# plus-rkwitt/flooder

Measured on AMD Instinct MI355X. Metric: M points×simplices/s (coverage sweep), higher is better.
Workload: dtype f32; 1 GPU; 1M-point 3D Gaussian, 1k landmarks, points_per_edge 30, max_dimension 3, fp32 coverage sweep (BASELINE.json configs[1]); points=1000000, landmarks=1000, top_simplices=6052, top_simplices_rank0=6052, swept_dimension=3, method=cell, parallelism=single GPU

## Files before the change

### flooder_amd/_native.py

```python

from __future__ import annotations

import ctypes
import os
from ctypes import c_char_p, c_float, c_int, c_int32, c_int64, c_uint32, c_void_p

_PKG_DIR = os.path.dirname(os.path.abspath(__file__))
LIB_PATH = os.environ.get("FLOODER_HIP_LIB") or os.path.join(_PKG_DIR, "libflooder_hip.so")



class _Block(ctypes.Structure):

    ABI = 1

    def __init__(self, **fields):
        super().__init__()
        self.size = ctypes.sizeof(self)
        self.abi = self.ABI
        known = {name for name, _ in self._fields_}
        for key, value in fields.items():
            if key not in known:
                raise TypeError(f"{type(self).__name__} has no field {key!r}")
            if value is not None and not isinstance(value, (int, float)):
# ... 8 lines not shown
        item = item.strip()
        if item:
            kind, name = item.split()
            out.append((name, kinds[kind]))
    return out


class FusedSweep(_Block):

    _fields_ = _fields("""u32 size; u32 abi; p pts_sorted; i64 n_pts; i32 dim; i32 k1; p nodes; p density_grid; p cloud_box;
        p verts; p weights; i32 R; i32 n_faces; i64 n_simplices; p memb; f32 alpha; i32 n_coarse; p coarse_rows; p parents;
        p face_bits; p face_slot; p d2_scratch; p flag_list; p flag_count; p flag_key; p flag_hist; p flag_sorted; p top;
        p top_list; p top_count; p simplex_weight; p plane_scratch; p wit_queue; p wit_item_list; p wit_stats;
        p cell_queue; p defer_list; p defer_c; p defer_ctl; p light_list; p heavy_list; p cell_stats; p finish_ctl;
        p hard_scratch; i32 hard_cap; i32 probed; p finish_stats; p wit_runs; i32 wit_run_len; i32 wit_n_runs;
        i32 planes_ready; i32 reserved""")


class SortedSweep(_Block):

    _fields_ = _fields("""u32 size; u32 abi; p pts_sorted; i64 n_pts; i32 dim; i32 k1; p nodes; p verts; p weights; i32 R;
        i32 n_faces; i64 n_simplices; p sample_order; p queue; p memb; p face_bits; p face_slot; p stats; p out_d2;
        i32 shard_rank; i32 shard_world""")


class FpsBatched(_Block):

    _fields_ = _fields("""u32 size; u32 abi; p pts; i64 n_pts; i32 dim; i32 ld; p pts_sorted; p order; i64 start; i32 n_lms;
        i32 reserved; p out_idx; p minsq; p bucket_box; p bucket_keys; p bucket_coord; p work_best; p work_rec; p work_ctr;
        p launches_out""")

# ... 102 lines not shown
                                             c_void_p]),
    "flooder_sweep_bvh_items_f32": (c_int, [c_void_p, c_int64, c_int, c_void_p, c_void_p, c_void_p, c_int, c_int,
                                            c_int64, c_void_p, c_void_p, c_void_p, c_void_p, c_int, c_void_p,
                                            c_void_p, c_void_p, c_void_p]),
    "flooder_sweep_cell_f32": (c_int, [c_void_p, c_int64, c_int, c_void_p, c_void_p, c_void_p, c_int, c_int,
                                       c_int64, c_float, c_void_p, c_void_p, c_void_p, c_void_p, c_void_p, c_void_p,
                                       c_void_p, c_void_p, c_void_p]),
    "flooder_density_grid_words": (c_int64, [c_int]),
    "flooder_density_grid_f32": (c_int, [c_void_p, c_int64, c_int, c_void_p, c_void_p, c_void_p]),
    "flooder_cloud_kind": (c_int, [c_void_p, c_int, c_void_p]),
    "flooder_wit_max_rows": (c_int, []),
    "flooder_wit_max_coarse": (c_int, []),
    "flooder_finish_single_tiles": (c_int, []),
    "flooder_finish_single_batches": (c_int, []),
    "flooder_face_values_f32": (c_int, [c_void_p, c_int64, c_void_p, c_void_p]),
    "flooder_simplex_weight_f32": (c_int, [c_void_p, c_int64, c_int, c_void_p, c_int, c_int64, c_void_p, c_void_p]),
    "flooder_simplex_planes_forget": (None, []),
    "flooder_simplex_prepare_f32": (c_int, [c_void_p, c_int64, c_int, c_void_p, c_int, c_int64, c_void_p, c_void_p, c_void_p,
                                            c_int64, c_void_p]),
    "flooder_selftest": (c_int, [c_void_p, c_void_p, c_void_p]),
    "flooder_fill_u32": (c_int, [c_void_p, c_int64, c_uint32, c_void_p]),
    "flooder_gather_rows_f64": (c_int, [c_void_p, c_int64, c_int, c_int, c_void_p, c_void_p, c_int64, c_void_p]),
    "flooder_sweep_bvh_f64": (c_int, [c_void_p, c_int64, c_int, c_void_p, c_void_p, c_void_p, c_int, c_int, c_int64,
                                      c_void_p, c_void_p, c_void_p]),
    "flooder_face_max_f64": (c_int, [c_void_p, c_int64, c_int, c_void_p, c_void_p, c_int, c_void_p, c_void_p, c_void_p]),
    "flooder_fps_bucket_count": (c_int64, [c_int64]),
    "flooder_fps_indexed_f32": (c_int, [c_void_p, c_int64, c_int, c_int, c_void_p, c_void_p, c_int, c_int64, c_void_p,
                                        c_void_p, c_void_p, c_void_p, c_void_p, c_void_p]),
    "flooder_fps_batched_max_points": (c_int64, []),
    "flooder_fps_batched_rec_words": (c_int64, [c_int64, c_int, c_int]),
# ... 108 lines not shown
```

### flooder_amd/core.py

```python

from __future__ import annotations

import ctypes
import itertools
import os
import weakref
import warnings
from numbers import Integral
from typing import Callable, Dict, List, NamedTuple, Optional, Tuple, Union

import numpy as np
import torch

from . import _native
from .simplex_tree import HAS_GUDHI, SimplexTree, delaunay_cells, delaunay_simplices

__all__ = ["flood_complex", "generate_landmarks", "generate_grid", "generate_uniform_weights",
           "SUPPORTED_DTYPES", "HAS_HIP_KERNELS", "PointIndex", "index_from_host"]

SUPPORTED_DTYPES = (torch.float32, torch.float64)
INF_BITS = 0x7F800000
CAND_ALIGN = 8
SWEEP_CHUNK = 2048
TILE_SAMPLES = 512
# ... 192 lines not shown
    n = simplex_vertices.shape[0]
    flat = torch.argmax(torch.cdist(simplex_vertices, simplex_vertices).flatten(1), dim=1)
    i0 = torch.div(flat, d + 1, rounding_mode="floor")
    i1 = flat - i0 * (d + 1)
    ar = torch.arange(n, device=simplex_vertices.device)
    centers = (simplex_vertices[ar, i0] + simplex_vertices[ar, i1]) / 2.0
    radii = torch.amax((simplex_vertices - centers.unsqueeze(1)).norm(dim=2), dim=1) \
        * (1.42 if d > 1 else 1.01) + 1e-3
    return centers, radii


_GRID_CACHE: Dict[tuple, tuple] = {}


def _grid_tables(points_per_edge: int, dim: int, device, dtype):
    key = (int(points_per_edge), int(dim), str(device), dtype, SAMPLE_UNITS)
    hit = _GRID_CACHE.get(key)
    if hit is None:
        weights, vertex_idxs, face_idxs = generate_grid(points_per_edge, dim, device, dtype)
        faces = _FaceTable(face_idxs, weights.shape[0], device)
        plan = SamplePlan(weights, faces) if torch.device(device).type == "cuda" else None
        v_np = [v.cpu().numpy() for v in vertex_idxs]
        if len(_GRID_CACHE) >= 16:
            _GRID_CACHE.clear()
        hit = _GRID_CACHE[key] = (weights, vertex_idxs, face_idxs, faces, plan, v_np)
    return hit


class _FaceTable:

    def __init__(self, face_idxs: Optional[List[torch.Tensor]], R: int, device):
# ... 496 lines not shown
        if n <= units[-1]:
            out.append(idx)
            continue
        P = X[idx]
        ax = int(np.argmax(P.max(axis=0) - P.min(axis=0)))
        idx = idx[np.argsort(P[:, ax], kind="stable")]
        unit = next((u for u in units if n > u), units[-1])
        n_left = (-(-n // unit) // 2) * unit
        if n_left <= 0 or n_left >= n:
            n_left = n // 2
        stack.append(idx[n_left:])
        stack.append(idx[:n_left])
    return np.concatenate(out)


WIT_MAX_COARSE = 256
WIT_MAX_ROWS = 8192
WIT_MIN_ROWS = 512
_WIT_PLAN_CACHE: Dict[tuple, Optional[tuple]] = {}


def witness_plan(weights: torch.Tensor, perm: np.ndarray) -> Optional[Tuple[np.ndarray, np.ndarray]]:
    w = weights.detach().cpu().numpy().astype(np.float64)
    R, k1 = w.shape
    if R < WIT_MIN_ROWS or R > WIT_MAX_ROWS or k1 < 2:
        return None
    key = (R, k1, hash(w.tobytes()), hash(np.asarray(perm).tobytes()))
    if key in _WIT_PLAN_CACHE:
        return _WIT_PLAN_CACHE[key]
    from scipy.spatial import cKDTree
# ... 68 lines not shown
    d = np.sqrt(((w - c64[:, None, :]) ** 2).sum(axis=2))
    rho = d.max(axis=1) * (1.0 + 1e-12)
    rho32 = rho.astype(np.float32)
    rho32 = np.where(rho32.astype(np.float64) < rho, np.nextafter(rho32, np.float32(np.inf)), rho32).astype(np.float32)
    sums = w32.astype(np.float64).sum(axis=1)
    if max(np.abs(sums - 1.0).max(), np.abs(c64.sum(axis=1) - 1.0).max()) > 0.5 * WIT_RUN_SUM_TOL:
        return None
    out = np.zeros((n, 8), dtype=np.uint32)
    out[:, :k1] = c32.view(np.uint32)
    out[:, 4] = np.bitwise_or.reduce(np.asarray(memb).view(np.uint32)[:n * run_len].reshape(n, run_len), axis=1)
    out[:, 5] = np.asarray(parents).view(np.uint32)[:n * run_len].reshape(n, run_len)[rows, d.argmin(axis=1)]
    out[:, 6] = rho32.view(np.uint32)
    return out


class SamplePlan:

    def __init__(self, weights: torch.Tensor, faces: _FaceTable):
        dev = weights.device
        self.R, self.k1 = weights.shape
        R = self.R
        perm = sample_order(weights)
        f_ptr = faces.ptr.cpu().numpy().astype(np.int64)
        f_rows = faces.rows.cpu().numpy().astype(np.int64)
        n_faces = faces.n_faces
        inv = np.empty(R, dtype=np.int64)
        inv[perm] = np.arange(R)
        self.inv = torch.as_tensor(inv, device=dev)
        self.w_perm = weights.to(torch.float32)[torch.as_tensor(perm, device=dev)].contiguous()
        self.rows_perm = self.inv[faces.rows.long()].to(torch.int32).contiguous()
        self.faces = faces
        self.memb_all = None
        if n_faces <= 32:
            memb_all = np.zeros(R, dtype=np.uint32)
            for f in range(n_faces):
                memb_all[inv[f_rows[f_ptr[f]:f_ptr[f + 1]]]] |= np.uint32(1 << f)
            self.memb_all = torch.as_tensor(memb_all.view(np.int32), device=dev)
        self._perm, self._weights, self._face_rows = perm, weights, (f_ptr, f_rows, inv)
        self._late_rows = self._wit = None
        self._late_built = self._wit_built = False
# ... 345 lines not shown
KNN_MERGE_WORKSPACE_BYTES = PROFILE_WORKSPACE_BYTES
SORTED_FUSED_FACES = False
BVH_SORTED_MIN_SAMPLES = 64 * 1024
EMPTY_CACHE_ABOVE_BYTES = 1 << 30
CELL_ALPHA = 1.35
FUSED_FACES = True
CELL_PROBE = True
SHARED_FACE_SLOTS = True
FINISH_HARD_CAP = 32768
CELL_DENSITY_GRID = True
CELL_SUPER = True
WIT_MIN_SIMPLICES = 1536
WIT_MAX_POINTS_PER_SIMPLEX = 400
CELL_WITNESS = True
WIT_RUNS = True


def _sweep_dimension_cell(index: PointIndex, verts: torch.Tensor, weights: torch.Tensor, faces: _FaceTable,
                          reduce_hook: Optional[Callable[[torch.Tensor], None]],
                          want_dist: bool = False, timer: Optional[_KernelTimer] = None,
                          stats: Optional[torch.Tensor] = None, plan: Optional[SamplePlan] = None,
                          face_slots: Optional[Tuple[torch.Tensor, int]] = None):
    lib = _native.load()
    dev = index.pts.device
    st = _native.current_stream_ptr(dev)
    S, k1, _ = verts.shape
    R = weights.shape[0]
    verts = verts.to(torch.float32).contiguous()
    plan = plan if plan is not None else SamplePlan(weights, faces)
    w_perm, rows_perm = plan.w_perm, plan.rows_perm
# ... 2 lines not shown
        return None if stats is None else stats[a:b]

    if S == 0:
        return (torch.empty((0, faces.n_faces), dtype=torch.float32, device=dev),
                torch.empty((0, R), dtype=torch.float32, device=dev) if want_dist else None)
    planes = torch.empty(24 * S, dtype=torch.float32, device=dev)
    if FUSED_FACES and not want_dist and reduce_hook is None and plan.memb_all is not None:
        F = faces.n_faces
        tiles = (R + 63) // 64
        slot_t, n_slots = face_slots if face_slots is not None else (None, S * F)
        CTL_FLAG_COUNT, CTL_DEFER, CTL_HIST = 1, 12, 48
        use_wit = (CELL_WITNESS and CELL_SUPER and CELL_PROBE and index.dim in (2, 3) and S >= WIT_MIN_SIMPLICES
                   and index.n <= WIT_MAX_POINTS_PER_SIMPLEX * S and plan.wit is not None)
        n_zeroed = ((1 if use_wit else 0) * QUEUE_WORDS + _native.CELL_QUEUE_WORDS + _native.FINISH_CTL_WORDS + 2 * S
                    + CTL_HIST + 8192 + n_slots)
        zeroed = (torch.empty if CELL_SUPER and SWEEP_PREPARE_FUSED else torch.zeros)(n_zeroed, dtype=torch.int32, device=dev)
        zeroed_all = zeroed
        if use_wit:
            qwit = zeroed[:QUEUE_WORDS]
            zeroed = zeroed[QUEUE_WORDS:]
        qbuf = zeroed[:_native.CELL_QUEUE_WORDS]
        fctl = zeroed[_native.CELL_QUEUE_WORDS:_native.CELL_QUEUE_WORDS + _native.FINISH_CTL_WORDS]
        zeroed = zeroed[_native.CELL_QUEUE_WORDS + _native.FINISH_CTL_WORDS:]
        top = zeroed[:2 * S].view(torch.int64)
        ctl = zeroed[2 * S:2 * S + CTL_HIST + 8192]
        face_bits = zeroed[2 * S + CTL_HIST + 8192:]
        hard = torch.empty(4 * FINISH_HARD_CAP, dtype=torch.int64, device=dev)
        top_list = torch.empty(S, dtype=torch.int32, device=dev)
        d2 = torch.empty((S, R), dtype=torch.int32, device=dev)
        flags = torch.empty((3, S * tiles), dtype=torch.int32, device=dev)
        chunks = (R + 255) // 256
        defer_list = torch.empty(5 * S * chunks, dtype=torch.int32, device=dev) if CELL_SUPER else None
        defer_c = torch.empty(5 * S * chunks, dtype=torch.float32, device=dev) if CELL_SUPER else None
        wgt = None
        split = torch.empty((2, S), dtype=torch.int32, device=dev) if CELL_SUPER else None
        if CELL_SUPER:
            wgt = torch.empty(S, dtype=torch.float32, device=dev)
            if SWEEP_PREPARE_FUSED:
                _native.check(lib.flooder_simplex_prepare_f32(_native.ptr(index.nodes), index.n, index.dim, _native.ptr(verts),
                                                              k1, S, _native.ptr(wgt), _native.ptr(planes),
                                                              _native.ptr(zeroed_all), n_zeroed, st),
# ... 4 lines not shown
        wst = stats[16:40] if use_wit and stats is not None and stats.numel() >= 40 else None
        blk = _native.FusedSweep(
            pts_sorted=index.pts, n_pts=index.n, dim=index.dim, k1=k1, nodes=index.nodes, density_grid=index.dens,
            cloud_box=index.box, verts=verts, weights=w_perm, R=R, n_faces=F, n_simplices=S, memb=plan.memb_all,
            alpha=float(CELL_ALPHA), face_bits=face_bits, face_slot=slot_t, d2_scratch=d2, flag_list=flags[0],
            flag_count=ctl[CTL_FLAG_COUNT:].data_ptr(), simplex_weight=wgt, plane_scratch=planes,
            cell_queue=qbuf.data_ptr(), defer_list=defer_list, defer_c=defer_c, cell_stats=sub(0, 9),
            finish_ctl=fctl.data_ptr(), hard_scratch=hard, hard_cap=FINISH_HARD_CAP, probed=1 if CELL_PROBE else 0,
            finish_stats=sub(9, 16))
        if CELL_PROBE:
            blk.flag_key, blk.flag_hist, blk.flag_sorted = flags[1].data_ptr(), ctl[CTL_HIST:].data_ptr(), flags[2].data_ptr()
            blk.top, blk.top_list = top.data_ptr(), top_list.data_ptr()
            blk.top_count = fctl[_native.FINISH_CTL_TOP_COUNT:].data_ptr()
        if CELL_SUPER:
            blk.defer_ctl, blk.light_list, blk.heavy_list = ctl[CTL_DEFER:].data_ptr(), split[0].data_ptr(), split[1].data_ptr()
        if use_wit:
            blk.n_coarse, blk.coarse_rows, blk.parents = plan.wit[2], plan.wit[0].data_ptr(), plan.wit[1].data_ptr()
            blk.wit_queue, blk.wit_item_list, blk.wit_stats = qwit.data_ptr(), split[0].data_ptr(), _native.ptr(wst) or None
            if WIT_RUNS and plan.wit_runs is not None:
                blk.wit_runs, blk.wit_run_len, blk.wit_n_runs = plan.wit_runs[0].data_ptr(), plan.wit_runs[1], plan.wit_runs[2]
        blk.planes_ready = 1 if CELL_SUPER and SWEEP_PREPARE_FUSED else 0
        with _span(timer, "sweep"):
            if use_wit:
                _native.check(lib.flooder_fused_witness(ctypes.byref(blk), st), "flooder_fused_witness")
                blk.planes_ready = 1
            _native.check(lib.flooder_fused_cell(ctypes.byref(blk), st), "flooder_fused_cell")
        with _span(timer, "fallback"):
            _native.check(lib.flooder_fused_finish(ctypes.byref(blk), st), "flooder_fused_finish")
        if stats is not None:
            c_d = ctl[CTL_DEFER:CTL_DEFER + _native.DEFER_CTL_WORDS].tolist()
            LAST_STATS.deferred_chunks = int(c_d[_native.DEFER_CTL_COUNT])
            LAST_STATS.light_heavy = (int(c_d[_native.DEFER_CTL_LIGHT]), int(c_d[_native.DEFER_CTL_HEAVY]))
            LAST_STATS.dense_tiles = int(c_d[_native.DEFER_CTL_TILE_COUNT])
            c_h = fctl[:_native.FINISH_CTL_QUEUES].tolist()
            LAST_STATS.hard_entries = (int(c_h[_native.FINISH_CTL_TOP_HARD_LEN]), int(c_h[_native.FINISH_CTL_REST_HARD_LEN]))
            LAST_STATS.finish_single_left = int(c_h[_native.FINISH_CTL_SINGLE_LEFT])
        out_face = torch.empty(n_slots if face_slots is not None else (S, F), dtype=torch.float32, device=dev)
        with _span(timer, "face_max"):
            _native.check(lib.flooder_face_values_f32(_native.ptr(face_bits), n_slots, _native.ptr(out_face), st),
                          "flooder_face_values_f32")
        return out_face, None

    ctl = torch.zeros(8 + 4 * QUEUE_WORDS, dtype=torch.int32, device=dev)
    qbuf = ctl[8:8 + 3 * QUEUE_WORDS]
    q_items = ctl[8 + 3 * QUEUE_WORDS:]
    d2 = torch.empty((S, R), dtype=torch.int32, device=dev)
    flags = torch.empty(S * ((R + 63) // 64), dtype=torch.int32, device=dev)
    with _span(timer, "sweep"):
        _native.check(lib.flooder_sweep_cell_f32(
            _native.ptr(index.pts), index.n, index.dim, _native.ptr(index.nodes), _native.ptr(verts),
            _native.ptr(w_perm), k1, R, S, float(CELL_ALPHA), qbuf.data_ptr(), _native.ptr(d2), _native.ptr(flags),
# ... 389 lines not shown
```

### flooder_amd/csrc/flood_cell.hip

```cpp

#include <type_traits>

#include "flood_common.hpp"
#include "flood_bvh.hpp"
#include "flood_planes.hpp"

using namespace flooder;

namespace {

constexpr int SPL_CHUNK = 4;
#ifndef FLOODER_CELL_CAPW
#define FLOODER_CELL_CAPW 480
#endif
#ifndef FLOODER_CELL_MAXLEAF
#define FLOODER_CELL_MAXLEAF 584
#endif
#ifndef FLOODER_CELL_WAVES
#define FLOODER_CELL_WAVES 4
#endif
#ifndef FLOODER_CELL_COMPACT
#define FLOODER_CELL_COMPACT 0
#endif
constexpr int CAPW = FLOODER_CELL_CAPW;
// ... 273 lines not shown
      const int gl = lfirst ? g : g - n_heavy_items;
      const int e = (TILES ? ARG(dl.tile_list) : ARG(dl.list))[gl];
      seeded = (e & 1) != 0;
      c_seed = (TILES ? ARG(dl.tile_c) : ARG(dl.c))[gl];
      s = (e >> 1) / chunks;
      q = (e >> 1) - s * chunks;
    } else {
      s = g / chunks;
      q = g - s * chunks;
    }
    s = wave_uniform(s);
    const int q_first = q;
    const float* vs = ARG(verts) + (int64_t)s * k1 * DIM;
    const int n_live = R;
    if (q * CHUNK >= n_live) continue;
    auto defer = [&](int qq, int seeded_flag, float c_next) {
      if (lane == 0) {
        const int pos = atomicAdd(ARG(dl.count), 1);
        ARG(dl.list)[pos] = (int)(((s * chunks + qq) << 1) | seeded_flag);
        ARG(dl.c)[pos] = c_next;
      }
    };
    PHASE(0);

    float p[SPL][DIM];
    float best[SPL];
    bool open[SPL];
    int row[SPL];
    float blo[DIM], bhi[DIM];
    auto make_samples = [&]() {
#pragma unroll
      for (int i = 0; i < SPL; ++i) {
        int slot = q * CHUNK + i * 64 + lane;
        open[i] = slot < n_live;
        if (slot >= n_live) slot = n_live - 1;
        const int r = slot;
        row[i] = r;
#pragma unroll
        for (int k = 0; k < DIM; ++k) p[i][k] = 0.f;
        if (k1 == 4) {
          const float4 w4 = *reinterpret_cast<const float4*>(weights + (int64_t)r * 4);
          const float wj[4] = {w4.x, w4.y, w4.z, w4.w};
#pragma unroll
          for (int j = 0; j < 4; ++j) {
#pragma unroll
            for (int k = 0; k < DIM; ++k) p[i][k] = __builtin_fmaf(wj[j], vs[j * DIM + k], p[i][k]);
          }
        } else {
          for (int j = 0; j < k1; ++j) {
            const float w = weights[(int64_t)r * k1 + j];
#pragma unroll
            for (int k = 0; k < DIM; ++k) p[i][k] = __builtin_fmaf(w, vs[j * DIM + k], p[i][k]);
// ... 24 lines not shown

    float slo[DIM + 1], shi[DIM + 1];
    {
      float mn[DIM], mx[DIM], dmn[DIM + 1], dmx[DIM + 1];
#pragma unroll
      for (int k = 0; k < DIM; ++k) { mn[k] = __builtin_inff(); mx[k] = -__builtin_inff(); }
#pragma unroll
      for (int f = 0; f <= DIM; ++f) { dmn[f] = __builtin_inff(); dmx[f] = -__builtin_inff(); }
      for (int sub = 0; sub < n_sub; ++sub) {
        q = q_first + sub;
        make_samples();
#pragma unroll
        for (int i = 0; i < SPL; ++i) {
#pragma unroll
          for (int k = 0; k < DIM; ++k) {
            mn[k] = __builtin_fminf(mn[k], p[i][k]);
            mx[k] = __builtin_fmaxf(mx[k], p[i][k]);
          }
#pragma unroll
          for (int f = 0; f <= DIM; ++f) {
            float dd = -po[f];
#pragma unroll
            for (int k = 0; k < DIM; ++k) dd = __builtin_fmaf(pn[f][k], p[i][k] - org[k], dd);
            dmn[f] = __builtin_fminf(dmn[f], dd);
            dmx[f] = __builtin_fmaxf(dmx[f], dd);
          }
        }
      }
#pragma unroll
      for (int k = 0; k < DIM; ++k) {
        blo[k] = wave_min_f32(mn[k]);
        bhi[k] = wave_max_f32(mx[k]);
      }
#pragma unroll
      for (int f = 0; f <= DIM; ++f) {
        slo[f] = wave_min_f32(dmn[f]);
        shi[f] = wave_max_f32(dmx[f]);
      }
    }
    float ext = 0.f, vol = 1.f;
// ... 158 lines not shown
    auto finalize = [&](bool seed_mode) {
    uint32_t* const out_d2 = ARG(out_d2);
    if (fused) {
      const FaceAcc acc = ARG(acc);
      uint32_t mb[SPL], um = 0u;
      bool fl_on[SPL];
      uint32_t fl_key[SPL];
#pragma unroll
      for (int i = 0; i < SPL; ++i) { fl_on[i] = false; fl_key[i] = 0u; }
      const int64_t my_slot = lane < acc.n_faces ? acc.slot_of(s, lane) : 0;
      const uint32_t my_fb = lane < acc.n_faces
                                 ? __hip_atomic_load(acc.face_bits + my_slot, __ATOMIC_RELAXED, __HIP_MEMORY_SCOPE_AGENT)
                                 : 0xffffffffu;
#pragma unroll
      for (int i = 0; i < SPL; ++i) {
        const bool settled = (q * CHUNK + i * 64 + lane < n_live) && !open[i];
        mb[i] = settled ? acc.memb[row[i]] : 0u;
        um |= mb[i];
      }
      um = wave_or_u32(um);
      while (um) {
        const int f = __builtin_ctz(um);
        um &= um - 1u;
        uint32_t v = 0u;
#pragma unroll
        for (int i = 0; i < SPL; ++i) {
          const uint32_t b = ((mb[i] >> f) & 1u) ? __float_as_uint(best[i]) : 0u;
          v = b > v ? b : v;
        }
        v = wave_max_u32(v);
        if (lane == f && v > my_fb) atomicMax(&acc.face_bits[my_slot], v);
// ... 869 lines not shown
int launch_simplex_planes(int dim, const float* verts, int k1, int64_t n_simplices, float* tab, hipStream_t st) {
  if (dim == 2)
    hipLaunchKernelGGL((simplex_planes_kernel<2>), dim3((unsigned)((n_simplices + 255) / 256)), dim3(256), 0, st, verts, k1,
                       n_simplices, tab);
  else if (dim == 3)
    hipLaunchKernelGGL((simplex_planes_kernel<3>), dim3((unsigned)((n_simplices + 255) / 256)), dim3(256), 0, st, verts, k1,
                       n_simplices, tab);
  else
    return fail(FLOODER_E_ARG, "simplex planes: only dim 2 and 3");
  return check_launch("simplex_planes");
}
}

namespace {

__global__ __launch_bounds__(1024) void split_simplices_kernel(const float* __restrict__ weight, int n, float limit,
                                                               float sparse_limit, int32_t* __restrict__ light,
                                                               int32_t* __restrict__ heavy, int32_t* __restrict__ counts) {
  __shared__ int s_cl[16], s_ch[16];
  __shared__ int s_sparse, s_act;
  const int lane = threadIdx.x & 63, wv = threadIdx.x >> 6;
  if (threadIdx.x == 0) { s_sparse = 0; s_act = 0; }
  __syncthreads();
  int mine = 0, act = 0;
  for (int i = threadIdx.x; i < n; i += 1024) {
    const float w = weight[i];
    mine += (w >= 0.f && w <= sparse_limit) ? 1 : 0;
    act += w >= 0.f ? 1 : 0;
  }
#pragma unroll
  for (int o = 32; o > 0; o >>= 1) {
    mine += __shfl_xor(mine, o);
    act += __shfl_xor(act, o);
// ... 21 lines not shown
    if (is_heavy) heavy[n_heavy + bh + __builtin_amdgcn_mbcnt_hi((uint32_t)(mh >> 32), __builtin_amdgcn_mbcnt_lo((uint32_t)mh, 0))] = i;
    n_light += tl;
    n_heavy += th;
    __syncthreads();
  }
  if (threadIdx.x == 0) { counts[0] = n_light; counts[1] = n_heavy; counts[2] = 1; }
}

constexpr int SPLIT_THREADS_LONG = 512;
constexpr int SPLIT_THREADS = 256;
constexpr int SPLIT_CLASSES = 9;
template <int NT>
__global__ __launch_bounds__(NT) void class_order_kernel(const float* __restrict__ weight, int n, float limit,
                                                               float sparse_limit, int runs_allowed, int reorder,
                                                               int32_t* __restrict__ light, int32_t* __restrict__ heavy,
                                                               int32_t* __restrict__ counts) {
  __shared__ int s_cnt[NT / 64][SPLIT_CLASSES + 1];
  constexpr int ID_LDS = 7680;
  __shared__ int s_id[ID_LDS];
  if (reorder) {
    n = counts[1];
    if (n > ID_LDS || n < 2 || counts[0] == 0) return;
    for (int i = threadIdx.x; i < n; i += NT) s_id[i] = heavy[i];
    __syncthreads();
  }
  constexpr int W_LDS = 7680;
  __shared__ float s_w[W_LDS];
  const bool staged = n <= W_LDS;
  if (staged) {
    for (int base = 0; base < n; base += NT * 8) {
      float v[8];
// ... 163 lines not shown
}

int flooder::fused_cell(const flooder_fused_sweep_t& a, void* stream) {
  if (a.n_simplices == 0 || a.R == 0) return FLOODER_OK;
  if (!a.memb || !a.face_bits || a.n_faces < 1 || a.n_faces > 32 || (a.top && (!a.top_list || !a.top_count)) ||
      (a.defer_list && (!a.defer_c || !a.defer_ctl)) ||
      (a.simplex_weight && (!a.defer_list || !a.light_list || !a.heavy_list)) || (a.flag_key && (!a.flag_hist || !a.top)) ||
      a.n_simplices > 0x7fffffffLL)
    return fail(FLOODER_E_ARG, "flooder_sweep_cell_faces_f32: bad argument");
  const float* const weight = a.simplex_weight;
  int32_t* const light = weight ? a.light_list : nullptr;
  int32_t* const heavy = weight ? a.heavy_list : nullptr;
  int32_t* const split = weight ? a.defer_ctl + FLOODER_DEFER_CTL_LIGHT : nullptr;
  const int n = (int)a.n_simplices;
  const hipStream_t st = (hipStream_t)stream;
  if (weight) {
    const bool long_queue = a.n_simplices * (int64_t)((a.R + 255) / 256) >= (int64_t)g_cell_super_min_chunks;
    if (long_queue && (g_cell_split_launches == 2 || a.n_simplices > 7680)) {
      hipLaunchKernelGGL(split_simplices_kernel, dim3(1), dim3(1024), 0, st, weight, n, (float)g_cell_super_weight,
                         (float)g_cell_super_sparse, light, heavy, split);
      if (g_cell_weight_classes)
        hipLaunchKernelGGL(class_order_kernel<SPLIT_THREADS>, dim3(1), dim3(SPLIT_THREADS), 0, st, weight, n,
                           (float)g_cell_super_weight, (float)g_cell_super_sparse, 2, 1, light, heavy, split);
    } else if (long_queue) {
      hipLaunchKernelGGL(class_order_kernel<SPLIT_THREADS_LONG>, dim3(1), dim3(SPLIT_THREADS_LONG), 0, st, weight, n,
                         (float)g_cell_super_weight, (float)g_cell_super_sparse, (g_cell_weight_classes ? 2 : 0) | 1 | 4, 0,
                         light, heavy, split);
    } else {
      hipLaunchKernelGGL(class_order_kernel<SPLIT_THREADS>, dim3(1), dim3(SPLIT_THREADS), 0, st, weight, n,
                         (float)g_cell_super_weight, (float)g_cell_super_sparse, g_cell_weight_classes ? 2 : 0, 0, light,
                         heavy, split);
    }
  }
  DeferList dl{a.defer_list, a.defer_c, a.defer_list ? a.defer_ctl + FLOODER_DEFER_CTL_COUNT : nullptr, light, heavy,
               split, g_cell_super_n0};
  if (a.defer_list) {
    const int64_t n_chunk_slots = a.n_simplices * (int64_t)((a.R + 255) / 256);
    dl.tile_list = a.defer_list + n_chunk_slots;
    dl.tile_c = a.defer_c + n_chunk_slots;
    dl.tile_count = a.defer_ctl + FLOODER_DEFER_CTL_TILE_COUNT;
  }
  return sweep_cell_entry(a,
                          FaceAcc{a.memb, a.face_bits, a.n_faces, reinterpret_cast<unsigned long long*>(a.top), a.top_list,
                                  a.top_count, a.face_slot, a.flag_key, a.flag_hist},
                          dl, "flooder_sweep_cell_faces_f32: bad argument", stream);
}

extern "C" {

int flooder_sweep_cell_f32(const float* pts_sorted, int64_t n_pts, int dim, const float* nodes,
                           const float* verts, const float* weights, int k1, int R, int64_t n_simplices,
                           float alpha, int32_t* queue, uint32_t* out_d2, int32_t* flag_list, int32_t* flag_count,
                           float* plane_scratch, const int32_t* density_grid, const float* cloud_box, uint64_t* stats,
                           void* stream) {
  flooder_fused_sweep_t a{};
  a.pts_sorted = pts_sorted; a.n_pts = n_pts; a.dim = dim; a.nodes = nodes; a.verts = verts; a.weights = weights;
  a.k1 = k1; a.R = R; a.n_simplices = n_simplices; a.alpha = alpha; a.cell_queue = queue; a.d2_scratch = out_d2;
  a.flag_list = flag_list; a.flag_count = flag_count; a.plane_scratch = plane_scratch; a.density_grid = density_grid;
  a.cloud_box = cloud_box; a.cell_stats = stats;
  return sweep_cell_entry(a, FaceAcc{nullptr, nullptr, 0, nullptr, nullptr, nullptr, nullptr},
// ... 56 lines not shown
```

### flooder_amd/csrc/flood_common.hpp

```cpp
#pragma once
#include <hip/hip_runtime.h>
#include <stdint.h>
#include <stdio.h>
#include <string.h>

#include "../../include/flooder_hip.h"

namespace flooder {

constexpr uint32_t INF_BITS = 0x7f800000u;

#define FLOODER_OPTION(name, def, lo, hi, desc) extern int g_##name;
#define FLOODER_OPTION_LIST(name, def, desc, ...) extern int g_##name;
#include "flood_options.def"
#undef FLOODER_OPTION
#undef FLOODER_OPTION_LIST
int launch_simplex_planes(int dim, const float* verts, int k1, int64_t n_simplices, float* tab, hipStream_t st);
char* err_buf();
int fail(int code, const char* msg);
int check_launch(const char* what);

__host__ __device__ constexpr int padded_dim(int dim) { return dim <= 2 ? 2 : (dim <= 4 ? 4 : 8); }

template <int DP>
// ... 162 lines not shown
  x |= dpp_move_u32<0x143, 0xC>(x);
  return (uint32_t)__builtin_amdgcn_readlane((int)x, 63);
}

constexpr uint32_t SETTLED_BIT = 0x80000000u;
struct FaceAcc {
  const uint32_t* memb;
  uint32_t* face_bits;
  int n_faces;
  unsigned long long* top;
  int32_t* top_list;
  int32_t* top_count;
  const int32_t* slot;
  uint32_t* flag_key = nullptr;
  int32_t* flag_hist = nullptr;
  __device__ __forceinline__ int64_t slot_of(int64_t s, int f) const {
    return slot ? (int64_t)slot[s * (int64_t)n_faces + f] : s * (int64_t)n_faces + f;
  }
};

template <template <int> class F, typename... Args>
int dispatch_dim(int dim, Args&&... args) {
  switch (dim) {
    case 1: return F<1>::run(args...);
    case 2: return F<2>::run(args...);
    case 3: return F<3>::run(args...);
    case 4: return F<4>::run(args...);
    case 5: return F<5>::run(args...);
    case 6: return F<6>::run(args...);
    case 7: return F<7>::run(args...);
    case 8: return F<8>::run(args...);
    default: return fail(FLOODER_E_ARG, "dim must be in 1..8");
  }
}
// ... 90 lines not shown
```

### flooder_amd/csrc/flood_finish.hip

```cpp

#include "flood_common.hpp"
#include "flood_bvh.hpp"
#include "flood_planes.hpp"

using namespace flooder;

namespace {

constexpr int SHORT_LIST = 1024;
#ifndef FLOODER_TOP_NODES
#define FLOODER_TOP_NODES 1024
#endif
#ifndef FLOODER_FINISH_PRIO_AFTER
#define FLOODER_FINISH_PRIO_AFTER 32
#endif
#ifndef FLOODER_FINISH_PRIO
#define FLOODER_FINISH_PRIO 3
#endif
#ifndef FLOODER_FINISH_WAVES
#define FLOODER_FINISH_WAVES 4
#endif
constexpr int TOP_NODES = FLOODER_TOP_NODES;

struct HardLists {
// ... 702 lines not shown
    const int c = s_cnt[b];
    if (c > 0) s_base[b] += atomicAdd(&cursor[b], c);
    s_cnt[b] = 0;
  }
  __syncthreads();
  for (int i = i0 + threadIdx.x; i < i1; i += 256) {
    const int b = (int)(flag_key[i] >> 19);
    flag_sorted[s_base[b] + atomicAdd(&s_cnt[b], 1)] = flag_list[i];
  }
}

__global__ void face_values_kernel(const uint32_t* __restrict__ bits, int64_t n, float* __restrict__ out) {
  const int64_t stride = (int64_t)gridDim.x * blockDim.x;
  for (int64_t i = (int64_t)blockIdx.x * blockDim.x + threadIdx.x; i < n; i += stride)
    out[i] = __builtin_sqrtf(__uint_as_float(bits[i]));
}

template <int DIM>
struct FinishOp {
  static int run(const flooder_fused_sweep_t& a, const Levels& lv, FaceAcc acc, hipStream_t st) {
    if constexpr (DIM != 2 && DIM != 3) {
      return fail(FLOODER_E_ARG, "flooder_finish_faces_f32: only dim 2 and 3");
    } else {
    int32_t* const ctl = a.finish_ctl;
    const int hard_cap = a.hard_cap;
    unsigned long long* top = reinterpret_cast<unsigned long long*>(a.top);
    unsigned long long* hard = reinterpret_cast<unsigned long long*>(a.hard_scratch);
    unsigned long long* stats = reinterpret_cast<unsigned long long*>(a.finish_stats);
    const int grid = g_bvh_grid;
    const bool wide = g_finish_wide_points > 0 && lv.count[0] * (int64_t)FLOODER_BVH_LEAF >= (int64_t)g_finish_wide_points;
// ... 92 lines not shown
  a.flag_sorted = flag_sorted; a.finish_ctl = ctl; a.top = top; a.top_list = top_list; a.probed = probed;
  a.d2_scratch = d2_scratch; a.memb = memb; a.n_faces = n_faces; a.face_bits = face_bits; a.face_slot = face_slot;
  a.hard_scratch = hard_scratch; a.hard_cap = hard_cap; a.finish_stats = stats;
  return fused_finish(a, stream);
}

int flooder_face_values_f32(const uint32_t* face_bits, int64_t n, float* out_face, void* stream) {
  if (n == 0) return FLOODER_OK;
  if (!face_bits || !out_face || n < 0) return fail(FLOODER_E_ARG, "flooder_face_values_f32: bad argument");
  int64_t blocks = (n + 255) / 256;
  if (blocks > 2048) blocks = 2048;
  hipLaunchKernelGGL(face_values_kernel, dim3((int)blocks), dim3(256), 0, (hipStream_t)stream, face_bits, n, out_face);
  return check_launch("face_values");
}

}

namespace {

constexpr int WFRONT = 256;

template <int DIM>
__global__ __launch_bounds__(256) void simplex_weight_kernel(const float* __restrict__ nodes, Levels lv,
                                                             const float* __restrict__ verts, int k1,
                                                             int64_t n_simplices, float* __restrict__ weight,
                                                             int weight_blocks, float* __restrict__ plane_tab,
                                                             int32_t* __restrict__ zero_buf, int64_t zero_words) {
  constexpr int DP = padded_dim(DIM);
  __shared__ int s_front[4][2][WFRONT];
  const int lane = threadIdx.x & 63, wv = threadIdx.x >> 6;
// ... 117 lines not shown
```

### include/flooder_hip.h

```cpp
#ifndef FLOODER_HIP_H
#define FLOODER_HIP_H

#include <stdint.h>

#ifdef __cplusplus
extern "C" {
#endif

#define FLOODER_ABI_VERSION 1

#define FLOODER_OK 0
#define FLOODER_E_ARG (-1)
#define FLOODER_E_LAUNCH (-2)
#define FLOODER_E_DEVICE (-3)

#define FLOODER_MAX_DIM 8
#define FLOODER_MAX_VERTS 9
#define FLOODER_CAND_ALIGN 8
#define FLOODER_SWEEP_CHUNK 2048
#define FLOODER_TILE_SAMPLES 512
#define FLOODER_BVH_LEAF 16
#define FLOODER_BVH_FANOUT 64
#define FLOODER_BVH_MAX_LEVELS 6
#define FLOODER_QUEUE_SHARDS 16
// ... 156 lines not shown
#define FLOODER_FINISH_CTL_WORDS (FLOODER_FINISH_CTL_QUEUES + 3 * FLOODER_QUEUE_WORDS)
#define FLOODER_DEFER_CTL_COUNT 0
#define FLOODER_DEFER_CTL_QUEUE 1
#define FLOODER_DEFER_CTL_LIGHT 2
#define FLOODER_DEFER_CTL_HEAVY 3
#define FLOODER_DEFER_CTL_SPLIT_DONE 4
#define FLOODER_DEFER_CTL_TILE_COUNT 6
#define FLOODER_DEFER_CTL_WORDS 8
#define FLOODER_CELL_QUEUE_RUNS 0
#define FLOODER_CELL_QUEUE_CHUNKS FLOODER_QUEUE_WORDS
#define FLOODER_CELL_QUEUE_TILES (2 * FLOODER_QUEUE_WORDS)
#define FLOODER_CELL_QUEUE_WORDS (3 * FLOODER_QUEUE_WORDS)
#define FLOODER_WIT_QUEUE_ITEM_COUNT (FLOODER_QUEUE_WORDS - 1)

int flooder_face_values_f32(const uint32_t* face_bits, int64_t n, float* out_face, void* stream);

int flooder_simplex_weight_f32(const float* nodes, int64_t n_pts, int dim, const float* verts, int k1,
                               int64_t n_simplices, float* weight, void* stream);

int flooder_simplex_prepare_f32(const float* nodes, int64_t n_pts, int dim, const float* verts, int k1,
                                int64_t n_simplices, float* weight, float* plane_scratch, int32_t* zero_buf,
                                int64_t zero_words, void* stream);
void flooder_simplex_planes_forget(void);

int flooder_selftest(const float* in64, float* out128, void* stream);

int flooder_fill_u32(uint32_t* buf, int64_t n, uint32_t value, void* stream);

int flooder_fps_f32(const float* pts, int64_t n_pts, int dim, int ld, int n_lms, int64_t start,
                    int64_t* out_idx, float* work_min, uint64_t* work_best, void* stream);
// ... 60 lines not shown
  float* defer_c;
  int32_t* defer_ctl;
  int32_t* light_list;
  int32_t* heavy_list;
  uint64_t* cell_stats;
  int32_t* finish_ctl;
  uint64_t* hard_scratch;
  int32_t hard_cap;
  int32_t probed;
  uint64_t* finish_stats;
  const uint32_t* wit_runs;
  int32_t wit_run_len;
  int32_t wit_n_runs;
  int32_t planes_ready;
  int32_t reserved;
} flooder_fused_sweep_t;

int flooder_fused_witness(const flooder_fused_sweep_t* p, void* stream);
int flooder_fused_cell(const flooder_fused_sweep_t* p, void* stream);
int flooder_fused_finish(const flooder_fused_sweep_t* p, void* stream);

typedef struct flooder_sorted_sweep_s {
  uint32_t size, abi;
  const float* pts_sorted;
  int64_t n_pts;
  int32_t dim;
  int32_t k1;
  const float* nodes;
  const float* verts;
  const float* weights;
// ... 154 lines not shown
```

Baseline: 6.217 million M points×simplices/s.

## Assign shared faces to one owner simplex and skip non-owned face samples

Grid rows are grouped by the smallest face that contains them. Each shared face gets a single owner simplex, chosen by atomicMax on a weight-based key inside the existing split/class-order launches. The cell sweep masks out rows on faces a simplex does not own and skips whole chunks or tiles that hold no owned faces. A new face-closure kernel then propagates maxima from sub-faces, so each face value still covers all of its boundary samples. This is meant to cut redundant sampling of faces shared between neighbouring simplices, at the cost of an owner pass, extra per-chunk mask loads and one more kernel.

```diff
diff --git a/flooder_amd/_native.py b/flooder_amd/_native.py
--- a/flooder_amd/_native.py
+++ b/flooder_amd/_native.py
@@ -46,7 +46,7 @@
         p top_list; p top_count; p simplex_weight; p plane_scratch; p wit_queue; p wit_item_list; p wit_stats;
         p cell_queue; p defer_list; p defer_c; p defer_ctl; p light_list; p heavy_list; p cell_stats; p finish_ctl;
         p hard_scratch; i32 hard_cap; i32 probed; p finish_stats; p wit_runs; i32 wit_run_len; i32 wit_n_runs;
-        i32 planes_ready; i32 reserved""")
+        i32 planes_ready; i32 reserved; p face_owner; p min_face; p chunk_faces; p tile_faces""")
 
 
 class SortedSweep(_Block):
@@ -179,6 +179,7 @@
     "flooder_finish_single_tiles": (c_int, []),
     "flooder_finish_single_batches": (c_int, []),
     "flooder_face_values_f32": (c_int, [c_void_p, c_int64, c_void_p, c_void_p]),
+    "flooder_face_closure_f32": (c_int, [c_void_p, c_void_p, c_void_p, c_int64, c_int, c_void_p, c_void_p]),
     "flooder_simplex_weight_f32": (c_int, [c_void_p, c_int64, c_int, c_void_p, c_int, c_int64, c_void_p, c_void_p]),
     "flooder_simplex_planes_forget": (None, []),
     "flooder_simplex_prepare_f32": (c_int, [c_void_p, c_int64, c_int, c_void_p, c_int, c_int64, c_void_p, c_void_p, c_void_p,
diff --git a/flooder_amd/core.py b/flooder_amd/core.py
--- a/flooder_amd/core.py
+++ b/flooder_amd/core.py
@@ -230,7 +230,7 @@
 
 
 def _grid_tables(points_per_edge: int, dim: int, device, dtype):
-    key = (int(points_per_edge), int(dim), str(device), dtype, SAMPLE_UNITS)
+    key = (int(points_per_edge), int(dim), str(device), dtype, SAMPLE_UNITS, bool(FACE_OWNER), bool(FACE_OWNER_GROUPED))
     hit = _GRID_CACHE.get(key)
     if hit is None:
         weights, vertex_idxs, face_idxs = generate_grid(points_per_edge, dim, device, dtype)
@@ -757,6 +757,56 @@
     return np.concatenate(out)
 
 
+def sample_order_grouped(weights: np.ndarray, group: np.ndarray) -> np.ndarray:
+    w = np.asarray(weights, dtype=np.float64)
+    R, k1 = w.shape
+    corners = np.eye(k1) - 1.0 / k1
+    X = w @ (corners @ np.linalg.qr(corners.T)[0][:, :k1 - 1])
+    out: List[np.ndarray] = []
+    pos = 0
+    for g in np.unique(group):
+        stack = [(np.nonzero(group == g)[0].astype(np.int64), pos)]
+        while stack:
+            idx, a = stack.pop()
+            n = idx.shape[0]
+            if n <= SAMPLE_UNITS[-1]:
+                out.append(idx)
+                continue
+            P = X[idx]
+            ax = int(np.argmax(P.max(axis=0) - P.min(axis=0)))
+            idx = idx[np.argsort(P[:, ax], kind="stable")]
+            n_left = n // 2
+            for u in SAMPLE_UNITS:
+                k0, k1_ = a // u + 1, -(-(a + n) // u) - 1
+                if k1_ >= k0:
+                    n_left = (k0 + (k1_ - k0 + 2) // 2 - 1) * u - a
+                    break
+            stack.append((idx[n_left:], a + n_left))
+            stack.append((idx[:n_left], a))
+        pos += int((group == g).sum())
+    return np.concatenate(out) if out else np.arange(R, dtype=np.int64)
+
+
+def row_groups(min_face: np.ndarray, sub_faces: np.ndarray, n_per_codim: List[int]) -> np.ndarray:
+    n1 = n_per_codim[1] if len(n_per_codim) > 1 else 0
+    group = min_face.astype(np.int64).copy()
+    small = group > n1
+    if small.any():
+        inside = (sub_faces[1:n1 + 1, None].astype(np.int64) >> min_face[None, small].astype(np.int64)) & 1
+        group[small] = 1 + inside.argmax(axis=0)
+    return group
+
+
+def _grouped_order_cached(w: np.ndarray, group: np.ndarray) -> np.ndarray:
+    key = (w.shape, hash(w.tobytes()), hash(group.tobytes()), SAMPLE_UNITS, "grouped")
+    hit = _SAMPLE_ORDER_CACHE.get(key)
+    if hit is None:
+        if len(_SAMPLE_ORDER_CACHE) >= 32:
+            _SAMPLE_ORDER_CACHE.clear()
+        hit = _SAMPLE_ORDER_CACHE[key] = sample_order_grouped(w, group)
+    return hit.copy()
+
+
 WIT_MAX_COARSE = 256
 WIT_MAX_ROWS = 8192
 WIT_MIN_ROWS = 512
@@ -855,6 +905,34 @@
     return out
 
 
+def face_lattice(weights: np.ndarray, f_ptr: np.ndarray, f_rows: np.ndarray) -> Optional[Tuple[np.ndarray, np.ndarray]]:
+    w = np.asarray(weights)
+    R, k1 = w.shape
+    F = len(f_ptr) - 1
+    if F > 32 or k1 > 31:
+        return None
+    supp = ((w != 0) * (1 << np.arange(k1))).sum(axis=1).astype(np.int64)
+    vset = np.array([np.bitwise_or.reduce(supp[f_rows[f_ptr[f]:f_ptr[f + 1]]]) if f_ptr[f + 1] > f_ptr[f] else 0
+                     for f in range(F)], dtype=np.int64)
+    if len(set(vset.tolist())) != F or (vset == 0).any():
+        return None
+    holds = (supp[:, None] & ~vset[None, :]) == 0
+    if not holds.any(axis=1).all():
+        return None
+    size = np.array([bin(int(v)).count("1") for v in vset])
+    min_face = np.where(holds, size[None, :], k1 + 1).argmin(axis=1).astype(np.uint8)
+    sub = (vset[None, :] & ~vset[:, None]) == 0
+    sub_faces = (sub * (1 << np.arange(F, dtype=np.int64))[None, :]).sum(axis=1).astype(np.uint32)
+    return min_face, sub_faces
+
+
+def _or_runs(bits: np.ndarray, run: int) -> np.ndarray:
+    n = (bits.shape[0] + run - 1) // run
+    pad = np.zeros(n * run, dtype=np.uint32)
+    pad[:bits.shape[0]] = bits
+    return np.bitwise_or.reduce(pad.reshape(n, run), axis=1)
+
+
 class SamplePlan:
 
     def __init__(self, weights: torch.Tensor, faces: _FaceTable):
@@ -865,6 +943,23 @@
         f_ptr = faces.ptr.cpu().numpy().astype(np.int64)
         f_rows = faces.rows.cpu().numpy().astype(np.int64)
         n_faces = faces.n_faces
+        self.min_face = self.chunk_faces = self.tile_faces = self.sub_faces = self.row_group = None
+        self.owner_order = False
+        if FACE_OWNER and n_faces <= 32 and self.k1 <= 8:
+            w_np = weights.detach().cpu().numpy()
+            lat = face_lattice(w_np, f_ptr, f_rows)
+            if lat is not None:
+                min_face, sub_faces = lat
+                if FACE_OWNER_GROUPED and len(f_ptr) > 2:
+                    group = row_groups(min_face, sub_faces, faces.n_per_codim)
+                    perm = _grouped_order_cached(w_np, group)
+                    self.row_group = group[perm]
+                bits = np.left_shift(np.uint32(1), min_face[perm].astype(np.uint32))
+                self.min_face = torch.as_tensor(np.ascontiguousarray(min_face[perm]), device=dev)
+                self.chunk_faces = torch.as_tensor(_or_runs(bits, 256).view(np.int32), device=dev)
+                self.tile_faces = torch.as_tensor(_or_runs(bits, 64).view(np.int32), device=dev)
+                self.sub_faces = torch.as_tensor(sub_faces.view(np.int32), device=dev)
+                self.owner_order = True
         inv = np.empty(R, dtype=np.int64)
         inv[perm] = np.arange(R)
         self.inv = torch.as_tensor(inv, device=dev)
@@ -1240,6 +1335,8 @@
 WIT_MAX_POINTS_PER_SIMPLEX = 400
 CELL_WITNESS = True
 WIT_RUNS = True
+FACE_OWNER = True
+FACE_OWNER_GROUPED = False
 
 
 def _sweep_dimension_cell(index: PointIndex, verts: torch.Tensor, weights: torch.Tensor, faces: _FaceTable,
@@ -1272,6 +1369,11 @@
                    and index.n <= WIT_MAX_POINTS_PER_SIMPLEX * S and plan.wit is not None)
         n_zeroed = ((1 if use_wit else 0) * QUEUE_WORDS + _native.CELL_QUEUE_WORDS + _native.FINISH_CTL_WORDS + 2 * S
                     + CTL_HIST + 8192 + n_slots)
+        use_owner = (FACE_OWNER and face_slots is not None and plan.owner_order and CELL_SUPER and SWEEP_PREPARE_FUSED
+                     and plan.sub_faces.numel() == F)
+        n_plain = n_zeroed
+        if use_owner:
+            n_zeroed += (n_zeroed & 1) + 3 * n_slots
         zeroed = (torch.empty if CELL_SUPER and SWEEP_PREPARE_FUSED else torch.zeros)(n_zeroed, dtype=torch.int32, device=dev)
         zeroed_all = zeroed
         if use_wit:
@@ -1282,7 +1384,8 @@
         zeroed = zeroed[_native.CELL_QUEUE_WORDS + _native.FINISH_CTL_WORDS:]
         top = zeroed[:2 * S].view(torch.int64)
         ctl = zeroed[2 * S:2 * S + CTL_HIST + 8192]
-        face_bits = zeroed[2 * S + CTL_HIST + 8192:]
+        face_bits = zeroed[2 * S + CTL_HIST + 8192:2 * S + CTL_HIST + 8192 + n_slots]
+        owner = zeroed_all[n_plain + (n_plain & 1):n_plain + (n_plain & 1) + 2 * n_slots] if use_owner else None
         hard = torch.empty(4 * FINISH_HARD_CAP, dtype=torch.int64, device=dev)
         top_list = torch.empty(S, dtype=torch.int32, device=dev)
         d2 = torch.empty((S, R), dtype=torch.int32, device=dev)
@@ -1317,6 +1420,9 @@
             blk.top_count = fctl[_native.FINISH_CTL_TOP_COUNT:].data_ptr()
         if CELL_SUPER:
             blk.defer_ctl, blk.light_list, blk.heavy_list = ctl[CTL_DEFER:].data_ptr(), split[0].data_ptr(), split[1].data_ptr()
+        if use_owner:
+            blk.face_owner, blk.min_face = owner.data_ptr(), plan.min_face.data_ptr()
+            blk.chunk_faces, blk.tile_faces = plan.chunk_faces.data_ptr(), plan.tile_faces.data_ptr()
         if use_wit:
             blk.n_coarse, blk.coarse_rows, blk.parents = plan.wit[2], plan.wit[0].data_ptr(), plan.wit[1].data_ptr()
             blk.wit_queue, blk.wit_item_list, blk.wit_stats = qwit.data_ptr(), split[0].data_ptr(), _native.ptr(wst) or None
@@ -1338,6 +1444,12 @@
             c_h = fctl[:_native.FINISH_CTL_QUEUES].tolist()
             LAST_STATS.hard_entries = (int(c_h[_native.FINISH_CTL_TOP_HARD_LEN]), int(c_h[_native.FINISH_CTL_REST_HARD_LEN]))
             LAST_STATS.finish_single_left = int(c_h[_native.FINISH_CTL_SINGLE_LEFT])
+        if use_owner:
+            out_face = zeroed_all[n_zeroed - n_slots:].view(torch.float32)
+            with _span(timer, "face_max"):
+                _native.check(lib.flooder_face_closure_f32(_native.ptr(face_bits), _native.ptr(slot_t), _native.ptr(plan.sub_faces),
+                                                           S, F, _native.ptr(out_face), st), "flooder_face_closure_f32")
+            return out_face, None
         out_face = torch.empty(n_slots if face_slots is not None else (S, F), dtype=torch.float32, device=dev)
         with _span(timer, "face_max"):
             _native.check(lib.flooder_face_values_f32(_native.ptr(face_bits), n_slots, _native.ptr(out_face), st),
diff --git a/flooder_amd/csrc/flood_cell.hip b/flooder_amd/csrc/flood_cell.hip
--- a/flooder_amd/csrc/flood_cell.hip
+++ b/flooder_amd/csrc/flood_cell.hip
@@ -311,6 +311,16 @@
     const float* vs = ARG(verts) + (int64_t)s * k1 * DIM;
     const int n_live = R;
     if (q * CHUNK >= n_live) continue;
+    const bool owned_rows = fused && ARG(acc.owner) != nullptr;
+    uint32_t own = 0xffffffffu;
+    if (owned_rows) {
+      const FaceAcc acc = ARG(acc);
+      own = acc.own_mask(s, lane);
+      const uint32_t* const run_faces = TILES ? acc.tile_faces : acc.chunk_faces;
+      uint32_t there = 0u;
+      for (int sub = 0; sub < n_sub; ++sub) there |= run_faces[q + sub];
+      if ((there & own) == 0u) continue;
+    }
     auto defer = [&](int qq, int seeded_flag, float c_next) {
       if (lane == 0) {
         const int pos = atomicAdd(ARG(dl.count), 1);
@@ -326,6 +336,7 @@
     int row[SPL];
     float blo[DIM], bhi[DIM];
     auto make_samples = [&]() {
+      const uint8_t* const min_face = owned_rows ? ARG(acc.min_face) : nullptr;
 #pragma unroll
       for (int i = 0; i < SPL; ++i) {
         int slot = q * CHUNK + i * 64 + lane;
@@ -333,6 +344,7 @@
         if (slot >= n_live) slot = n_live - 1;
         const int r = slot;
         row[i] = r;
+        if (min_face) open[i] = open[i] && ((own >> min_face[r]) & 1u) != 0u;
 #pragma unroll
         for (int k = 0; k < DIM; ++k) p[i][k] = 0.f;
         if (k1 == 4) {
@@ -387,16 +399,16 @@
         for (int i = 0; i < SPL; ++i) {
 #pragma unroll
           for (int k = 0; k < DIM; ++k) {
-            mn[k] = __builtin_fminf(mn[k], p[i][k]);
-            mx[k] = __builtin_fmaxf(mx[k], p[i][k]);
+            mn[k] = __builtin_fminf(mn[k], open[i] ? p[i][k] : __builtin_inff());
+            mx[k] = __builtin_fmaxf(mx[k], open[i] ? p[i][k] : -__builtin_inff());
           }
 #pragma unroll
           for (int f = 0; f <= DIM; ++f) {
             float dd = -po[f];
 #pragma unroll
             for (int k = 0; k < DIM; ++k) dd = __builtin_fmaf(pn[f][k], p[i][k] - org[k], dd);
-            dmn[f] = __builtin_fminf(dmn[f], dd);
-            dmx[f] = __builtin_fmaxf(dmx[f], dd);
+            dmn[f] = __builtin_fminf(dmn[f], open[i] ? dd : __builtin_inff());
+            dmx[f] = __builtin_fmaxf(dmx[f], open[i] ? dd : -__builtin_inff());
           }
         }
       }
@@ -585,7 +597,8 @@
                                  : 0xffffffffu;
 #pragma unroll
       for (int i = 0; i < SPL; ++i) {
-        const bool settled = (q * CHUNK + i * 64 + lane < n_live) && !open[i];
+        bool settled = (q * CHUNK + i * 64 + lane < n_live) && !open[i];
+        if (acc.owner) settled = settled && ((own >> acc.min_face[row[i]]) & 1u) != 0u;
         mb[i] = settled ? acc.memb[row[i]] : 0u;
         um |= mb[i];
       }
@@ -1485,9 +1498,34 @@
 
 namespace {
 
+struct OwnerJob {
+  unsigned long long* owner = nullptr;
+  const int32_t* slot = nullptr;
+  int n_faces = 0;
+};
+__device__ __forceinline__ void choose_owners(const OwnerJob& oj, const float* __restrict__ weight, int n, int block,
+                                              int n_blocks, int tid, int nt) {
+  const int64_t total = (int64_t)n * oj.n_faces;
+  for (int64_t t = (int64_t)block * nt + tid; t < total; t += (int64_t)n_blocks * nt) {
+    const int s = (int)(t / oj.n_faces);
+    if (t - (int64_t)s * oj.n_faces == 0) continue;
+    atomicMax(&oj.owner[oj.slot[t]], owner_key(s, weight[s]));
+  }
+}
+inline int owner_blocks(const OwnerJob& oj, int n, int nt) {
+  if (!oj.owner) return 0;
+  const int64_t b = ((int64_t)n * oj.n_faces + 4 * nt - 1) / (4 * nt);
+  return (int)(b < 1 ? 1 : (b > 1024 ? 1024 : b));
+}
+
 __global__ __launch_bounds__(1024) void split_simplices_kernel(const float* __restrict__ weight, int n, float limit,
                                                                float sparse_limit, int32_t* __restrict__ light,
-                                                               int32_t* __restrict__ heavy, int32_t* __restrict__ counts) {
+                                                               int32_t* __restrict__ heavy, int32_t* __restrict__ counts,
+                                                               OwnerJob oj) {
+  if (blockIdx.x > 0) {
+    choose_owners(oj, weight, n, (int)blockIdx.x - 1, (int)gridDim.x - 1, (int)threadIdx.x, 1024);
+    return;
+  }
   __shared__ int s_cl[16], s_ch[16];
   __shared__ int s_sparse, s_act;
   const int lane = threadIdx.x & 63, wv = threadIdx.x >> 6;
@@ -1539,7 +1577,11 @@
 __global__ __launch_bounds__(NT) void class_order_kernel(const float* __restrict__ weight, int n, float limit,
                                                                float sparse_limit, int runs_allowed, int reorder,
                                                                int32_t* __restrict__ light, int32_t* __restrict__ heavy,
-                                                               int32_t* __restrict__ counts) {
+                                                               int32_t* __restrict__ counts, OwnerJob oj) {
+  if (blockIdx.x > 0) {
+    choose_owners(oj, weight, n, (int)blockIdx.x - 1, (int)gridDim.x - 1, (int)threadIdx.x, NT);
+    return;
+  }
   __shared__ int s_cnt[NT / 64][SPLIT_CLASSES + 1];
   constexpr int ID_LDS = 7680;
   __shared__ int s_id[ID_LDS];
@@ -1733,22 +1775,26 @@
   int32_t* const split = weight ? a.defer_ctl + FLOODER_DEFER_CTL_LIGHT : nullptr;
   const int n = (int)a.n_simplices;
   const hipStream_t st = (hipStream_t)stream;
+  if (a.face_owner && (!weight || !a.face_slot || !a.min_face || !a.chunk_faces || !a.tile_faces))
+    return fail(FLOODER_E_ARG, "flooder_fused_cell: face_owner needs simplex_weight, face_slot, min_face, chunk_faces and tile_faces");
+  OwnerJob oj;
+  if (a.face_owner) { oj.owner = reinterpret_cast<unsigned long long*>(a.face_owner); oj.slot = a.face_slot; oj.n_faces = a.n_faces; }
   if (weight) {
     const bool long_queue = a.n_simplices * (int64_t)((a.R + 255) / 256) >= (int64_t)g_cell_super_min_chunks;
     if (long_queue && (g_cell_split_launches == 2 || a.n_simplices > 7680)) {
-      hipLaunchKernelGGL(split_simplices_kernel, dim3(1), dim3(1024), 0, st, weight, n, (float)g_cell_super_weight,
-                         (float)g_cell_super_sparse, light, heavy, split);
+      hipLaunchKernelGGL(split_simplices_kernel, dim3(1 + owner_blocks(oj, n, 1024)), dim3(1024), 0, st, weight, n,
+                         (float)g_cell_super_weight, (float)g_cell_super_sparse, light, heavy, split, oj);
       if (g_cell_weight_classes)
         hipLaunchKernelGGL(class_order_kernel<SPLIT_THREADS>, dim3(1), dim3(SPLIT_THREADS), 0, st, weight, n,
-                           (float)g_cell_super_weight, (float)g_cell_super_sparse, 2, 1, light, heavy, split);
+                           (float)g_cell_super_weight, (float)g_cell_super_sparse, 2, 1, light, heavy, split, OwnerJob{});
     } else if (long_queue) {
-      hipLaunchKernelGGL(class_order_kernel<SPLIT_THREADS_LONG>, dim3(1), dim3(SPLIT_THREADS_LONG), 0, st, weight, n,
-                         (float)g_cell_super_weight, (float)g_cell_super_sparse, (g_cell_weight_classes ? 2 : 0) | 1 | 4, 0,
-                         light, heavy, split);
+      hipLaunchKernelGGL(class_order_kernel<SPLIT_THREADS_LONG>, dim3(1 + owner_blocks(oj, n, SPLIT_THREADS_LONG)),
+                         dim3(SPLIT_THREADS_LONG), 0, st, weight, n, (float)g_cell_super_weight, (float)g_cell_super_sparse,
+                         (g_cell_weight_classes ? 2 : 0) | 1 | 4, 0, light, heavy, split, oj);
     } else {
-      hipLaunchKernelGGL(class_order_kernel<SPLIT_THREADS>, dim3(1), dim3(SPLIT_THREADS), 0, st, weight, n,
-                         (float)g_cell_super_weight, (float)g_cell_super_sparse, g_cell_weight_classes ? 2 : 0, 0, light,
-                         heavy, split);
+      hipLaunchKernelGGL(class_order_kernel<SPLIT_THREADS>, dim3(1 + owner_blocks(oj, n, SPLIT_THREADS)), dim3(SPLIT_THREADS), 0,
+                         st, weight, n, (float)g_cell_super_weight, (float)g_cell_super_sparse, g_cell_weight_classes ? 2 : 0,
+                         0, light, heavy, split, oj);
     }
   }
   DeferList dl{a.defer_list, a.defer_c, a.defer_list ? a.defer_ctl + FLOODER_DEFER_CTL_COUNT : nullptr, light, heavy,
@@ -1759,10 +1805,12 @@
     dl.tile_c = a.defer_c + n_chunk_slots;
     dl.tile_count = a.defer_ctl + FLOODER_DEFER_CTL_TILE_COUNT;
   }
-  return sweep_cell_entry(a,
-                          FaceAcc{a.memb, a.face_bits, a.n_faces, reinterpret_cast<unsigned long long*>(a.top), a.top_list,
-                                  a.top_count, a.face_slot, a.flag_key, a.flag_hist},
-                          dl, "flooder_sweep_cell_faces_f32: bad argument", stream);
+  FaceAcc acc{a.memb, a.face_bits, a.n_faces, reinterpret_cast<unsigned long long*>(a.top), a.top_list,
+              a.top_count, a.face_slot, a.flag_key, a.flag_hist};
+  if (a.face_owner) {
+    acc.owner = oj.owner; acc.min_face = a.min_face; acc.chunk_faces = a.chunk_faces; acc.tile_faces = a.tile_faces;
+  }
+  return sweep_cell_entry(a, acc, dl, "flooder_sweep_cell_faces_f32: bad argument", stream);
 }
 
 extern "C" {
diff --git a/flooder_amd/csrc/flood_common.hpp b/flooder_amd/csrc/flood_common.hpp
--- a/flooder_amd/csrc/flood_common.hpp
+++ b/flooder_amd/csrc/flood_common.hpp
@@ -200,10 +200,29 @@
   const int32_t* slot;
   uint32_t* flag_key = nullptr;
   int32_t* flag_hist = nullptr;
+  const unsigned long long* owner = nullptr;
+  const uint8_t* min_face = nullptr;
+  const uint32_t* chunk_faces = nullptr;
+  const uint32_t* tile_faces = nullptr;
+  __device__ __forceinline__ uint32_t own_mask(int64_t s, int lane) const {
+    bool mine = false;
+    if (lane > 0 && lane < n_faces) {
+      const unsigned long long k =
+          __hip_atomic_load(owner + slot[s * (int64_t)n_faces + lane], __ATOMIC_RELAXED, __HIP_MEMORY_SCOPE_AGENT);
+      mine = (uint32_t)k == ~(uint32_t)s;
+    }
+    return (uint32_t)__ballot(mine) | 1u;
+  }
   __device__ __forceinline__ int64_t slot_of(int64_t s, int f) const {
     return slot ? (int64_t)slot[s * (int64_t)n_faces + f] : s * (int64_t)n_faces + f;
   }
 };
+
+__device__ __forceinline__ unsigned long long owner_key(int s, float w) {
+  const uint32_t wb = __float_as_uint(w) < 0x7f800000u ? __float_as_uint(w) : 0x7f800000u;
+  const uint32_t hi = w < 0.f ? 0xffffffffu : 0x7fffffffu - wb;
+  return ((unsigned long long)hi << 32) | (unsigned long long)(~(uint32_t)s);
+}
 
 template <template <int> class F, typename... Args>
 int dispatch_dim(int dim, Args&&... args) {
diff --git a/flooder_amd/csrc/flood_finish.hip b/flooder_amd/csrc/flood_finish.hip
--- a/flooder_amd/csrc/flood_finish.hip
+++ b/flooder_amd/csrc/flood_finish.hip
@@ -740,6 +740,25 @@
   const int64_t stride = (int64_t)gridDim.x * blockDim.x;
   for (int64_t i = (int64_t)blockIdx.x * blockDim.x + threadIdx.x; i < n; i += stride)
     out[i] = __builtin_sqrtf(__uint_as_float(bits[i]));
+}
+
+template <int W>
+__global__ __launch_bounds__(256) void face_closure_kernel(const uint32_t* __restrict__ bits, const int32_t* __restrict__ slot,
+                                                           const uint32_t* __restrict__ sub_faces, int64_t n_simplices,
+                                                           int n_faces, float* __restrict__ out) {
+  const int lane = threadIdx.x & 63;
+  const int f = lane & (W - 1), base = lane & ~(W - 1);
+  const int64_t s = ((int64_t)blockIdx.x * blockDim.x + threadIdx.x) / W;
+  const bool on = s < n_simplices && f < n_faces;
+  const int64_t my_slot = on ? (int64_t)slot[s * n_faces + f] : 0;
+  const uint32_t raw = on ? bits[my_slot] : 0u;
+  const uint32_t sub = on ? sub_faces[f] : 0u;
+  uint32_t v = raw;
+  for (int g = 0; g < n_faces; ++g) {
+    const uint32_t t = (uint32_t)__shfl((int)raw, base + g);
+    v = ((sub >> g) & 1u) && t > v ? t : v;
+  }
+  if (on) out[my_slot] = __builtin_sqrtf(__uint_as_float(v));
 }
 
 template <int DIM>
@@ -862,6 +881,23 @@
   return check_launch("face_values");
 }
 
+int flooder_face_closure_f32(const uint32_t* face_bits, const int32_t* face_slot, const uint32_t* sub_faces,
+                             int64_t n_simplices, int n_faces, float* out_face, void* stream) {
+  if (n_simplices == 0) return FLOODER_OK;
+  if (!face_bits || !face_slot || !sub_faces || !out_face || n_simplices < 0 || n_faces < 1 || n_faces > 32)
+    return fail(FLOODER_E_ARG, "flooder_face_closure_f32: bad argument");
+  const int w = n_faces <= 16 ? 16 : 32;
+  const int64_t blocks = (n_simplices * w + 255) / 256;
+  if (blocks > 0x7fffffffLL) return fail(FLOODER_E_ARG, "flooder_face_closure_f32: too many simplices");
+  if (w == 16)
+    hipLaunchKernelGGL(face_closure_kernel<16>, dim3((unsigned)blocks), dim3(256), 0, (hipStream_t)stream, face_bits, face_slot,
+                       sub_faces, n_simplices, n_faces, out_face);
+  else
+    hipLaunchKernelGGL(face_closure_kernel<32>, dim3((unsigned)blocks), dim3(256), 0, (hipStream_t)stream, face_bits, face_slot,
+                       sub_faces, n_simplices, n_faces, out_face);
+  return check_launch("face_closure");
+}
+
 }
 
 namespace {
diff --git a/include/flooder_hip.h b/include/flooder_hip.h
--- a/include/flooder_hip.h
+++ b/include/flooder_hip.h
@@ -194,6 +194,9 @@
 #define FLOODER_WIT_QUEUE_ITEM_COUNT (FLOODER_QUEUE_WORDS - 1)
 
 int flooder_face_values_f32(const uint32_t* face_bits, int64_t n, float* out_face, void* stream);
+
+int flooder_face_closure_f32(const uint32_t* face_bits, const int32_t* face_slot, const uint32_t* sub_faces,
+                             int64_t n_simplices, int n_faces, float* out_face, void* stream);
 
 int flooder_simplex_weight_f32(const float* nodes, int64_t n_pts, int dim, const float* verts, int k1,
                                int64_t n_simplices, float* weight, void* stream);
@@ -284,6 +287,10 @@
   int32_t wit_n_runs;
   int32_t planes_ready;
   int32_t reserved;
+  uint64_t* face_owner;
+  const uint8_t* min_face;
+  const uint32_t* chunk_faces;
+  const uint32_t* tile_faces;
 } flooder_fused_sweep_t;
 
 int flooder_fused_witness(const flooder_fused_sweep_t* p, void* stream);
```

Result: faster. 6.515 million M points×simplices/s, median of 6 (+4.8%).
